# ApricityXX/PaddlePaddle

Hardware: AMD Instinct MI355X
Metric: tokens/sec GPT-3-13B sharding-3 + ResNet50 img/s, at 1/2/4/8 MI355X (higher is better)
Workload: dtype bf16; 1 GPU; model=GPT-3 13B (h5120 L40 a40 ffn20480 V50304), global_batch=16, seq_len=2048, micro_batch=4, accum_steps=4, parallelism=sharding_stage3_degree1, recompute=False, fused_head_ce=False, paired_wgrad=False, optimizer=AdamW fp32-master fused HIP, amp=O2 bf16, allocator=native auto-growth best-fit

## Files before the change

### csrc/dispatch/dispatch_gen.inc

```

extern "C" int pa_rms_norm_fwd(void*, void*, void*, void*, int64_t, int64_t, float, int, void*);
static PyObject* w_pa_rms_norm_fwd(PyObject*, PyObject* const* a, Py_ssize_t n) {
  if (n != 9) return bad_nargs("pa_rms_norm_fwd", 9, n);
  void* a0;
  if (!arg_ptr(a[0], &a0)) return nullptr;
  void* a1;
  if (!arg_ptr(a[1], &a1)) return nullptr;
  void* a2;
  if (!arg_ptr(a[2], &a2)) return nullptr;
  void* a3;
  if (!arg_ptr(a[3], &a3)) return nullptr;
  int64_t a4;
  if (!arg_i64(a[4], &a4)) return nullptr;
  int64_t a5;
  if (!arg_i64(a[5], &a5)) return nullptr;
  float a6;
  if (!arg_f32(a[6], &a6)) return nullptr;
  int a7;
  if (!arg_i32(a[7], &a7)) return nullptr;
  void* a8;
  if (!arg_ptr(a[8], &a8)) return nullptr;
  return PyLong_FromLongLong(static_cast<long long>(pa_rms_norm_fwd(a0, a1, a2, a3, a4, a5, a6, a7, a8)));
}
extern "C" int pa_rms_norm_bwd(void*, void*, void*, void*, void*, void*, int64_t, int64_t, int, void*);
// ... 116 lines not shown
  void* a2;
  if (!arg_ptr(a[2], &a2)) return nullptr;
  void* a3;
  if (!arg_ptr(a[3], &a3)) return nullptr;
  int a4;
  if (!arg_i32(a[4], &a4)) return nullptr;
  int64_t a5;
  if (!arg_i64(a[5], &a5)) return nullptr;
  int a6;
  if (!arg_i32(a[6], &a6)) return nullptr;
  int a7;
  if (!arg_i32(a[7], &a7)) return nullptr;
  void* a8;
  if (!arg_ptr(a[8], &a8)) return nullptr;
  return PyLong_FromLongLong(static_cast<long long>(pa_reduce_parts(a0, a1, a2, a3, a4, a5, a6, a7, a8)));
}
extern "C" int pa_softmax_fwd(void*, void*, int64_t, int64_t, int, void*);
static PyObject* w_pa_softmax_fwd(PyObject*, PyObject* const* a, Py_ssize_t n) {
  if (n != 6) return bad_nargs("pa_softmax_fwd", 6, n);
  void* a0;
  if (!arg_ptr(a[0], &a0)) return nullptr;
  void* a1;
  if (!arg_ptr(a[1], &a1)) return nullptr;
  int64_t a2;
  if (!arg_i64(a[2], &a2)) return nullptr;
  int64_t a3;
  if (!arg_i64(a[3], &a3)) return nullptr;
  int a4;
  if (!arg_i32(a[4], &a4)) return nullptr;
  void* a5;
// ... 2460 lines not shown
  if (!arg_ptr(a[6], &a6)) return nullptr;
  return PyLong_FromLongLong(static_cast<long long>(pa_moe_route(a0, a1, a2, a3, a4, a5, a6)));
}
extern "C" int pa_version();
static PyObject* w_pa_version(PyObject*, PyObject* const* a, Py_ssize_t n) {
  if (n != 0) return bad_nargs("pa_version", 0, n);
  return PyLong_FromLongLong(static_cast<long long>(pa_version()));
}
static PyMethodDef kGenMethods[] = {
    {"pa_rms_norm_fwd", reinterpret_cast<PyCFunction>(reinterpret_cast<void (*)(void)>(w_pa_rms_norm_fwd)), METH_FASTCALL, nullptr},
    {"pa_rms_norm_bwd", reinterpret_cast<PyCFunction>(reinterpret_cast<void (*)(void)>(w_pa_rms_norm_bwd)), METH_FASTCALL, nullptr},
    {"pa_rms_norm_bwd_res", reinterpret_cast<PyCFunction>(reinterpret_cast<void (*)(void)>(w_pa_rms_norm_bwd_res)), METH_FASTCALL, nullptr},
    {"pa_layer_norm_fwd", reinterpret_cast<PyCFunction>(reinterpret_cast<void (*)(void)>(w_pa_layer_norm_fwd)), METH_FASTCALL, nullptr},
    {"pa_layer_norm_bwd", reinterpret_cast<PyCFunction>(reinterpret_cast<void (*)(void)>(w_pa_layer_norm_bwd)), METH_FASTCALL, nullptr},
    {"pa_reduce_parts", reinterpret_cast<PyCFunction>(reinterpret_cast<void (*)(void)>(w_pa_reduce_parts)), METH_FASTCALL, nullptr},
    {"pa_softmax_fwd", reinterpret_cast<PyCFunction>(reinterpret_cast<void (*)(void)>(w_pa_softmax_fwd)), METH_FASTCALL, nullptr},
    {"pa_softmax_bwd", reinterpret_cast<PyCFunction>(reinterpret_cast<void (*)(void)>(w_pa_softmax_bwd)), METH_FASTCALL, nullptr},
    {"pa_softmax_ce_fwd", reinterpret_cast<PyCFunction>(reinterpret_cast<void (*)(void)>(w_pa_softmax_ce_fwd)), METH_FASTCALL, nullptr},
    {"pa_softmax_ce_bwd", reinterpret_cast<PyCFunction>(reinterpret_cast<void (*)(void)>(w_pa_softmax_ce_bwd)), METH_FASTCALL, nullptr},
    {"pa_ce_slice_fwd", reinterpret_cast<PyCFunction>(reinterpret_cast<void (*)(void)>(w_pa_ce_slice_fwd)), METH_FASTCALL, nullptr},
    {"pa_ce_slice_bwd", reinterpret_cast<PyCFunction>(reinterpret_cast<void (*)(void)>(w_pa_ce_slice_bwd)), METH_FASTCALL, nullptr},
    {"pa_gelu_fwd", reinterpret_cast<PyCFunction>(reinterpret_cast<void (*)(void)>(w_pa_gelu_fwd)), METH_FASTCALL, nullptr},
    {"pa_gelu_bwd", reinterpret_cast<PyCFunction>(reinterpret_cast<void (*)(void)>(w_pa_gelu_bwd)), METH_FASTCALL, nullptr},
    {"pa_swiglu_fwd", reinterpret_cast<PyCFunction>(reinterpret_cast<void (*)(void)>(w_pa_swiglu_fwd)), METH_FASTCALL, nullptr},
    {"pa_swiglu_bwd", reinterpret_cast<PyCFunction>(reinterpret_cast<void (*)(void)>(w_pa_swiglu_bwd)), METH_FASTCALL, nullptr},
    {"pa_bias_gelu_fwd", reinterpret_cast<PyCFunction>(reinterpret_cast<void (*)(void)>(w_pa_bias_gelu_fwd)), METH_FASTCALL, nullptr},
    {"pa_rope_fwd", reinterpret_cast<PyCFunction>(reinterpret_cast<void (*)(void)>(w_pa_rope_fwd)), METH_FASTCALL, nullptr},
    {"pa_rope_rows", reinterpret_cast<PyCFunction>(reinterpret_cast<void (*)(void)>(w_pa_rope_rows)), METH_FASTCALL, nullptr},
    {"pa_adamw_multi", reinterpret_cast<PyCFunction>(reinterpret_cast<void (*)(void)>(w_pa_adamw_multi)), METH_FASTCALL, nullptr},
    {"pa_adam_hyper_step", reinterpret_cast<PyCFunction>(reinterpret_cast<void (*)(void)>(w_pa_adam_hyper_step)), METH_FASTCALL, nullptr},
// ... 81 lines not shown
```

### csrc/kernels/common.h

```cpp
#pragma once
#include <hip/hip_runtime.h>
#include <hip/hip_bf16.h>
#include <hip/hip_fp16.h>
#include <stdint.h>

#define PA_EXPORT extern "C" __attribute__((visibility("default")))

namespace pa {

constexpr int kWave = 64;

enum DType : int { kF32 = 0, kF16 = 1, kBF16 = 2 };

using bf16 = __hip_bfloat16;
using f16 = __half;

template <typename T> struct Vec8;
template <> struct Vec8<bf16> { using type = uint4; };
template <> struct Vec8<f16> { using type = uint4; };

__device__ __forceinline__ float to_f(float x) { return x; }
__device__ __forceinline__ float to_f(bf16 x) { return __bfloat162float(x); }
__device__ __forceinline__ float to_f(f16 x) { return __half2float(x); }

// ... 100 lines not shown
template <int NT>
__device__ __forceinline__ float block_max(float v, float* smem) {
  v = wave_max(v);
  const int w = threadIdx.x >> 6, l = threadIdx.x & 63;
  __syncthreads();
  if (l == 0) smem[w] = v;
  __syncthreads();
  float r = -INFINITY;
#pragma unroll
  for (int i = 0; i < NT / 64; ++i) r = fmaxf(r, smem[i]);
  return r;
}

__host__ __device__ inline int64_t cdiv(int64_t a, int64_t b) { return (a + b - 1) / b; }

}

#define PA_DISPATCH_DTYPE(code, T, ...)                   \
  switch (code) {                                         \
    case pa::kF32: { using T = float; __VA_ARGS__; break; } \
    case pa::kF16: { using T = pa::f16; __VA_ARGS__; break; } \
    case pa::kBF16: { using T = pa::bf16; __VA_ARGS__; break; } \
    default: return 2;                                    \
  }

#define PA_CHECK_LAUNCH() do { hipError_t e_ = hipGetLastError(); if (e_ != hipSuccess) return 1; } while (0)
```

### csrc/kernels/linear_epi.hip

```cpp
#include "common.h"

using namespace pa;

namespace {

constexpr float kSqrt2OverPi = 0.7978845608028654f;
constexpr float kCoeff = 0.044715f;

__device__ __forceinline__ float gelu_tanh_grad(float x) { return gelu_tanh_grad_fast(x); }

__device__ __forceinline__ uint32_t hash32(uint64_t seed, uint64_t i) {
  uint64_t z = seed + (i + 1) * 0x9E3779B97F4A7C15ull;
  z = (z ^ (z >> 30)) * 0xBF58476D1CE4E5B9ull;
  z = (z ^ (z >> 27)) * 0x94D049BB133111EBull;
  z ^= z >> 31;
  return (uint32_t)(z >> 32);
}
__device__ __forceinline__ bool keep(uint64_t seed, uint64_t i, uint32_t thresh) { return hash32(seed, i) >= thresh; }

template <typename T>
__global__ __launch_bounds__(256) void colsum_partial_k(const T* __restrict__ x, float* __restrict__ part, int64_t rows,
                                                        int64_t cols, int nparts) {
  const int64_t c = ((int64_t)blockIdx.x * 256 + threadIdx.x) * 8;
  if (c >= cols) return;
  float acc[8] = {0, 0, 0, 0, 0, 0, 0, 0};
  for (int64_t r = blockIdx.y; r < rows; r += nparts) {
    float v[8];
    load8<T>(x + r * cols + c, v);
#pragma unroll
    for (int j = 0; j < 8; ++j) acc[j] += v[j];
  }
  store8<float>(part + (int64_t)blockIdx.y * cols + c, acc);
}
// ... 143 lines not shown
  const int dtype = dtype_acc & 0xff, acc = (dtype_acc >> 8) & 1;
  const int np = nparts_for(rows);
  dim3 g1((unsigned)cdiv(cols, 2048), (unsigned)np), g2((unsigned)cdiv(cols, 64));
  PA_DISPATCH_DTYPE(dtype, T, {
    hipLaunchKernelGGL((bias_gelu_bwd_k<T>), g1, dim3(256), 0, st, (const T*)h, (const T*)b, (const T*)dy, (T*)dh,
                       ws, rows, cols, np);
    hipLaunchKernelGGL((fold_partials_k<T>), g2, dim3(256), 0, st, ws, (T*)db, cols, np, acc);
  });
  PA_CHECK_LAUNCH();
  return 0;
}

PA_EXPORT int pa_dropout_add_fwd(const void* x, const void* res, void* out, int64_t n, float p, uint64_t seed,
                                 int dtype, hipStream_t st) {
  const int64_t nvec = n / 8;
  const uint32_t thresh = (uint32_t)fminf(p * 4294967296.0f, 4294967295.0f);
  const float scale = p < 1.f ? 1.f / (1.f - p) : 0.f;
  PA_DISPATCH_DTYPE(dtype, T, hipLaunchKernelGGL((dropout_add_k<T>), dim3(grid_ew(nvec)), dim3(256), 0, st,
                                                 (const T*)x, (const T*)res, (T*)out, nvec, seed, thresh, scale));
  PA_CHECK_LAUNCH();
  return 0;
}

PA_EXPORT int pa_dropout_bwd(const void* dy, void* dx, int64_t n, float p, uint64_t seed, int dtype, hipStream_t st) {
  const int64_t nvec = n / 8;
  const uint32_t thresh = (uint32_t)fminf(p * 4294967296.0f, 4294967295.0f);
  const float scale = p < 1.f ? 1.f / (1.f - p) : 0.f;
  PA_DISPATCH_DTYPE(dtype, T, hipLaunchKernelGGL((dropout_bwd_k<T>), dim3(grid_ew(nvec)), dim3(256), 0, st,
                                                 (const T*)dy, (T*)dx, nvec, seed, thresh, scale));
  PA_CHECK_LAUNCH();
  return 0;
}

PA_EXPORT int pa_dropout_bwd_colsum(const void* dy, void* dx, float* ws, int64_t rows, int64_t cols, float p,
                                    uint64_t seed, int dtype, hipStream_t st) {
  if (cols % 8) return 1;
  const uint32_t thresh = (uint32_t)fminf(p * 4294967296.0f, 4294967295.0f);
  const float scale = p < 1.f ? 1.f / (1.f - p) : 0.f;
  const int np = nparts_for(rows);
  dim3 g1((unsigned)cdiv(cols, 2048), (unsigned)np);
  PA_DISPATCH_DTYPE(dtype, T, hipLaunchKernelGGL((dropout_bwd_colsum_k<T>), g1, dim3(256), 0, st, (const T*)dy, (T*)dx,
                                                 ws, rows, cols, np, seed, thresh, scale));
  PA_CHECK_LAUNCH();
  return 0;
}

PA_EXPORT int64_t pa_colsum_nparts(int64_t rows) { return nparts_for(rows); }

PA_EXPORT int pa_fold_partials(const float* ws, void* out, int64_t cols, int64_t nparts, int dtype_acc,
                               hipStream_t st) {
  const int dtype = dtype_acc & 0xff, acc = (dtype_acc >> 8) & 1;
  dim3 g2((unsigned)cdiv(cols, 64));
  PA_DISPATCH_DTYPE(dtype, T, hipLaunchKernelGGL((fold_partials_k<T>), g2, dim3(256), 0, st, ws, (T*)out, cols,
// ... 5 lines not shown
```

### csrc/kernels/norm.hip

```cpp
#include "common.h"

using namespace pa;

namespace {

template <typename T, int VPL, bool LN>
__global__ __launch_bounds__(256) void norm_fwd_rows(const T* __restrict__ x, const T* __restrict__ w,
                                                     const T* __restrict__ b, T* __restrict__ y,
                                                     float* __restrict__ mean_out, float* __restrict__ rstd_out,
                                                     int64_t rows, int64_t cols, float eps) {
  const int lane = threadIdx.x & 63;
  const int64_t row = (int64_t)blockIdx.x * 4 + (threadIdx.x >> 6);
  if (row >= rows) return;
  const T* xr = x + row * cols;
  const float sh = LN ? to_f(xr[0]) : 0.f;
  float v[VPL][8];
  float s = 0.f;
#pragma unroll
  for (int k = 0; k < VPL; ++k) {
    const int64_t e = ((int64_t)k * 64 + lane) * 8;
    if (e < cols) {
      load8<T>(xr + e, v[k]);
    } else {
#pragma unroll
// ... 234 lines not shown
  else if (vpl <= 3) PA_BWD(3);
  else if (vpl <= 4) PA_BWD(4);
  else if (vpl <= 6) PA_BWD(6);
  else hipLaunchKernelGGL((norm_bwd_dx_wide<T, LN>), dim3((unsigned)rows), block, 0, st, DY, X, W, mean, rstd, DX, rows, cols,
                          RES);
#undef PA_BWD
  PA_CHECK_LAUNCH();
  if (dw_part) {
    dim3 g2((unsigned)cdiv(cols, 2048), (unsigned)nparts);
    hipLaunchKernelGGL((norm_bwd_wb<T, LN>), g2, block, 0, st, DY, X, mean, rstd, dw_part, db_part, rows, cols, nparts);
    PA_CHECK_LAUNCH();
  }
  return 0;
}

}

PA_EXPORT int pa_rms_norm_fwd(const void* x, const void* w, void* y, float* rstd, int64_t rows, int64_t cols,
                              float eps, int dtype, hipStream_t st) {
  PA_DISPATCH_DTYPE(dtype, T, return (launch_fwd<T, false>(x, w, nullptr, y, nullptr, rstd, rows, cols, eps, st)));
  return 0;
}

PA_EXPORT int pa_rms_norm_bwd(const void* dy, const void* x, const void* w, const float* rstd, void* dx,
                              float* dw_part, int64_t rows, int64_t cols, int dtype_np, hipStream_t st) {
  const int dtype = dtype_np & 0xff, nparts = dtype_np >> 8;
  PA_DISPATCH_DTYPE(dtype, T,
                    return (launch_bwd<T, false>(dy, x, w, nullptr, rstd, dx, w ? dw_part : nullptr, nullptr, rows,
                                                 cols, nparts > 0 ? nparts : 1, st)));
  return 0;
// ... 71 lines not shown
```

### paddlepaddle_amd/framework/flags.py

```python
from __future__ import annotations

import os

_FLAGS = {
    "FLAGS_check_nan_inf": False,
    "FLAGS_check_nan_inf_level": 0,
    "FLAGS_use_hip_kernels": True,
    "FLAGS_cudnn_deterministic": False,
    "FLAGS_embedding_deterministic": 0,
    "FLAGS_fraction_of_gpu_memory_to_use": 0.92,
    "FLAGS_allocator_strategy": "auto_growth",
    "FLAGS_eager_delete_tensor_gb": 0.0,
    "FLAGS_use_cuda_graph": False,
    "FLAGS_enable_pir_api": False,
    "FLAGS_print_ir": False,
    "FLAGS_call_stack_level": 1,
    "FLAGS_dp_bucket_mb": 128,
    "FLAGS_sharding_bucket_mb": 256,
    "FLAGS_pir_native_interpreter": True,
    "FLAGS_eager_backward_engine": "native",
    "FLAGS_weight_only_dequant_cache_mb": 4096,
    "FLAGS_fused_grad_accumulation": True,
    "FLAGS_static_native_executor": "auto",
    "FLAGS_gemm_backend": "auto",
    "FLAGS_sharding_stage3_keep_params": "auto",
    "FLAGS_conv_per_direction": True,
    "FLAGS_conv_bn_fusion": True,
    "FLAGS_use_autotune": True,
    "FLAGS_autotune_range_begin": 0,
    "FLAGS_autotune_range_end": 1 << 30,
    "FLAGS_layout_autotune": False,
    "FLAGS_dataloader_autotune": False,
    "FLAGS_dataloader_tuning_steps": 8,
    "FLAGS_static_engine_native": "auto",
    "FLAGS_linear_wt_cache_mb": 0,
}

for _k in list(_FLAGS):
    if _k in os.environ:
        _v = os.environ[_k]
        _d = _FLAGS[_k]
        if isinstance(_d, bool):
            _FLAGS[_k] = _v.lower() in ("1", "true", "yes")
        elif isinstance(_d, int):
            _FLAGS[_k] = int(_v)
        elif isinstance(_d, float):
            _FLAGS[_k] = float(_v)
        else:
            _FLAGS[_k] = _v

# ... 25 lines not shown
```

### paddlepaddle_amd/models/gpt.py

```python
from __future__ import annotations

import dataclasses
import math

import torch

from .. import nn
from ..framework.tensor import Tensor, _wrap
from ..nn import functional as F
from ..nn import initializer as I
from .. import ops as _ops


@dataclasses.dataclass
class GPTConfig:
    vocab_size: int = 50304
    hidden_size: int = 5120
    num_hidden_layers: int = 40
    num_attention_heads: int = 40
    intermediate_size: int = 20480
    max_position_embeddings: int = 2048
    hidden_dropout_prob: float = 0.1
    attention_probs_dropout_prob: float = 0.0
    initializer_range: float = 0.02
# ... 71 lines not shown
        init = I.Normal(0.0, cfg.initializer_range)
        if cfg.tensor_parallel_degree > 1:
            self.word_embeddings = _tp().VocabParallelEmbedding(cfg.vocab_size, cfg.hidden_size,
                                                                weight_attr=nn.ParamAttr(initializer=init))
        else:
            self.word_embeddings = nn.Embedding(cfg.vocab_size, cfg.hidden_size,
                                                weight_attr=nn.ParamAttr(initializer=init))
        self.position_embeddings = nn.Embedding(cfg.max_position_embeddings, cfg.hidden_size,
                                                weight_attr=nn.ParamAttr(initializer=init))
        self.dropout = nn.Dropout(cfg.hidden_dropout_prob)

        self.sp = _use_sp(cfg)
        if self.sp:
            _sp().mark_sequence_parallel(self.position_embeddings.weight)

    def forward(self, input_ids, position_ids=None):
        if self.sp:
            return self._forward_sp(input_ids, position_ids)
        if position_ids is None:
            S = input_ids.shape[-1]
            position_ids = _wrap(torch.arange(S, device=input_ids._t.device).unsqueeze(0))
        x = self.word_embeddings(input_ids)._t
        pe = self.position_embeddings(position_ids)._t
        p = self.dropout.p if self.training else 0.0
        return _wrap(_ops.dropout_add(x + pe, None, p, self.training))

    def _forward_sp(self, input_ids, position_ids):
        sp = _sp()
        ids = input_ids._t
        B, S = ids.shape[0], ids.shape[-1]
        emb = self.word_embeddings.local_lookup(ids).reshape(B * S, -1)
        x = sp.reduce_scatter_tokens(emb)
        r0, r1 = sp.token_block_range(B * S)
        if position_ids is None:
            pos = torch.arange(r0, r1, device=ids.device) % S
        else:
            pos = position_ids._t.expand(B, S).reshape(-1)[r0:r1]
        pe = torch.nn.functional.embedding(pos, self.position_embeddings.weight._t)
        p = self.dropout.p if self.training else 0.0
# ... 45 lines not shown
        return fn(qkv)

    def _forward_sp(self, x):
        sp = _sp()
        B, S = self.bs
        w, b = self.qkv_proj.weight._t, self.qkv_proj.bias._t
        t = x._t if x._t.dtype == w.dtype else x._t.to(w.dtype)
        qkv = sp.column_sp_linear(t, w, b)
        qkv = qkv.view(B, S, self.local_heads, 3, self.head_dim)
        o = _ops.flash_attention_qkvpacked(qkv, causal=True, dropout=self.attn_dropout, training=self.training)
        o = o.reshape(B * S, self.local_heads * self.head_dim)
        y = sp.row_sp_linear(o, self.out_proj.weight._t)
        return _wrap(y + self.out_proj.bias._t)


def _tracing():
    from ..framework.trace_hook import _active_program
    return _active_program() is not None


class GPTMLP(nn.Layer):
    def __init__(self, cfg: GPTConfig):
        super().__init__()
        h, f = cfg.hidden_size, cfg.intermediate_size
        init = I.Normal(0.0, cfg.initializer_range)
        out_init = I.Normal(0.0, cfg.initializer_range / math.sqrt(2.0 * cfg.num_hidden_layers))
        self.tp = cfg.tensor_parallel_degree
        if self.tp > 1:
            tp = _tp()
            self.linear1 = tp.ColumnParallelLinear(h, f, weight_attr=nn.ParamAttr(initializer=init), has_bias=True,
# ... 32 lines not shown


class GPTDecoderLayer(nn.Layer):
    def __init__(self, cfg: GPTConfig):
        super().__init__()
        self.norm1 = nn.LayerNorm(cfg.hidden_size, epsilon=cfg.layer_norm_eps)
        self.self_attn = GPTAttention(cfg)
        self.norm2 = nn.LayerNorm(cfg.hidden_size, epsilon=cfg.layer_norm_eps)
        self.mlp = GPTMLP(cfg)
        self.dropout1 = nn.Dropout(cfg.hidden_dropout_prob)
        self.dropout2 = nn.Dropout(cfg.hidden_dropout_prob)
        if _use_sp(cfg):
            _sp().mark_sequence_parallel(self.norm1.weight, self.norm1.bias, self.norm2.weight, self.norm2.bias)

    def _ln(self, norm, x):
        r, h = _ops.layer_norm_residual(x._t, norm.weight._t, norm.bias._t, norm._epsilon)
        return r, _wrap(h)

    def _attn(self, h):
        return _gpt_attn(self, h)

    def forward(self, x):
        p = self.dropout1.p if self.training else 0.0
        r, h = self._ln(self.norm1, x)
        x = _wrap(_ops.dropout_add(self._attn(h)._t, r, p, self.training))
        r, h = self._ln(self.norm2, x)
        x = _wrap(_ops.dropout_add(self.mlp(h)._t, r, p, self.training))
        return x


def _gpt_attn(layer, h):
    g = getattr(layer, "_rc", None)
    if g == "full_attn":
        from ..distributed.fleet.recompute import recompute
        return recompute(layer.self_attn, h)
    layer.self_attn._rc_core = g == "core_attn"
    return layer.self_attn(h)


class GPTModel(nn.Layer):
    def __init__(self, cfg: GPTConfig):
        super().__init__()
        self.config = cfg
        self.embeddings = GPTEmbeddings(cfg)
        self.layers = nn.LayerList([GPTDecoderLayer(cfg) for _ in range(cfg.num_hidden_layers)])
        self.norm = nn.LayerNorm(cfg.hidden_size, epsilon=cfg.layer_norm_eps)
        if _use_sp(cfg):
            _sp().mark_sequence_parallel(self.norm.weight, self.norm.bias)

    def forward(self, input_ids, position_ids=None):
        if _use_sp(self.config):
            bs = (input_ids.shape[0], input_ids.shape[-1])
            for layer in self.layers:
                layer.self_attn.bs = bs
        x = self.embeddings(input_ids, position_ids)
        rc = self.config.use_recompute and self.training
        gran = self.config.recompute_granularity
        skip = set(self.config.no_recompute_layers or ())
        if rc:
            from ..distributed.fleet.recompute import recompute
        for i, layer in enumerate(self.layers):
            on = rc and i not in skip
            if on and gran == "full":
                x = recompute(layer, x)
            else:
                layer._rc = gran if on else None
                x = layer(x)
        return self.norm(x)


class GPTForPretraining(nn.Layer):
    def __init__(self, cfg: GPTConfig):
        super().__init__()
        self.config = cfg
        self.gpt = GPTModel(cfg)
        if not cfg.tie_word_embeddings:
            self.lm_head_weight = self.create_parameter([cfg.vocab_size // max(cfg.tensor_parallel_degree, 1),
                                                         cfg.hidden_size],
                                                        default_initializer=I.Normal(0.0, cfg.initializer_range))

    def forward(self, input_ids, position_ids=None, labels=None, loss_mask=None, ignore_index=-100):
        h = self.gpt(input_ids, position_ids)
# ... 42 lines not shown
```

### paddlepaddle_amd/ops/__init__.py

```python
from __future__ import annotations

from .activation import gelu, silu, swiglu, softmax, bias_gelu
from .norm import rms_norm, rms_norm_residual, layer_norm, layer_norm_residual, add_rms_norm
from .loss import softmax_cross_entropy
from .attention import flash_attention, attention_bhsd, flash_attention_qkvpacked, qkv_rope_attention, attention_reference, paged_decode_attention, dense_decode_attention
from .rope import apply_rotary, decode_rope_cache
from .linear import fused_linear, colsum, linear_nt, ffn_gelu
from .lm_head import lm_head_cross_entropy
from .dropout import dropout_add
from . import optim
from ._loader import has as has_kernel, hip_enabled_for, LIB_PATH
from .bn import batch_norm_act_nhwc
from . import conv, gemm, dwconv, quant
```

### paddlepaddle_amd/ops/_sigs.py

```python
import ctypes

_vp = ctypes.c_void_p
_i64 = ctypes.c_int64
_i32 = ctypes.c_int
_f32 = ctypes.c_float
_u64 = ctypes.c_uint64

SIGS = {
    "pa_rms_norm_fwd": [_vp, _vp, _vp, _vp, _i64, _i64, _f32, _i32, _vp],
    "pa_rms_norm_bwd": [_vp, _vp, _vp, _vp, _vp, _vp, _i64, _i64, _i32, _vp],
    "pa_rms_norm_bwd_res": [_vp, _vp, _vp, _vp, _vp, _vp, _vp, _i64, _i64, _i32, _vp],
    "pa_layer_norm_fwd": [_vp, _vp, _vp, _vp, _vp, _vp, _i64, _i64, _f32, _i32, _vp],
    "pa_layer_norm_bwd": [_vp, _vp, _vp, _vp, _vp, _vp, _vp, _vp, _vp, _i64, _i64, _i32, _vp],
    "pa_reduce_parts": [_vp, _vp, _vp, _vp, _i32, _i64, _i32, _i32, _vp],
    "pa_softmax_fwd": [_vp, _vp, _i64, _i64, _i32, _vp],
    "pa_softmax_bwd": [_vp, _vp, _vp, _i64, _i64, _i32, _vp],
    "pa_softmax_ce_fwd": [_vp, _vp, _vp, _vp, _i64, _i64, _i64, _i32, _vp],
    "pa_softmax_ce_bwd": [_vp, _vp, _vp, _vp, _vp, _i64, _i64, _i64, _i32, _vp],
    "pa_ce_slice_fwd": [_vp, _vp, _vp, _vp, _i64, _i64, _i64, _i32, _vp],
    "pa_ce_slice_bwd": [_vp, _vp, _vp, _vp, _vp, _i64, _i64, _i64, _i64, _i32, _vp],
    "pa_gelu_fwd": [_vp, _vp, _i64, _i32, _i32, _vp],
    "pa_gelu_bwd": [_vp, _vp, _vp, _i64, _i32, _i32, _vp],
    "pa_swiglu_fwd": [_vp, _vp, _vp, _i64, _i64, _i64, _i32, _vp],
    "pa_swiglu_bwd": [_vp, _vp, _vp, _vp, _vp, _i64, _i64, _i64, _i32, _vp],
    "pa_bias_gelu_fwd": [_vp, _vp, _vp, _i64, _i64, _i32, _vp],
    "pa_rope_fwd": [_vp, _vp, _vp, _vp, _i64, _i64, _i64, _i64, _i32, _i32, _vp],
    "pa_rope_rows": [_vp, _i64, _vp, _vp, _vp, _i64, _i64, _i64, _i64, _i64, _i32, _i32, _vp],
    "pa_adamw_multi": [_vp, _vp, _i64, _vp, _f32, _f32, _f32, _f32, _f32, _f32, _f32, _vp, _vp],
    "pa_adam_hyper_step": [_vp, _f32, _f32, _vp],
# ... 81 lines not shown
    "pa_bn_bwd_apply_nhwc": [_vp] * 6 + [_i64, _i32, _i32, _vp, _vp],
    "pa_bn_pre_ws": [_i32, _i32],
    "pa_bn_bwd_nhwc_pre": [_vp] * 9 + [_i32, _vp, _vp, _i64, _i32, _i32, _vp, _vp],
    "pa_bn_fwd_nhwc_pre": [_vp] * 10 + [_i32, _vp, _vp, _vp, _i64, _i32, _f32, _f32, _i32, _vp],
    "pa_add_rms_norm_fwd": [_vp, _vp, _vp, _vp, _vp, _i64, _i64, _f32, _i32, _vp],
    "pa_decode_rope_cache": [_vp, _i64, _vp, _vp, _vp, _vp, _vp, _vp, _i32, _i32, _i32, _i32, _i64, _i32, _vp],
    "pa_maxpool_nhwc_fwd": [_vp, _vp, _vp] + [_i32] * 10 + [_vp],
    "pa_maxpool_nhwc_bwd": [_vp, _vp, _vp] + [_i32] * 10 + [_vp],
    "pa_grouped_gemm": [_i32, _vp, _vp, _vp, _vp, _vp, _vp, _i32, _i64, _i32, _i32, _i32, _i64, _i64, _i64, _i32,
                        _vp],
    "pa_moe_route": [_vp, _i32, _i32, _vp, _vp, _vp, _vp],
    "pa_version": [],
}

RET_I64 = {"pa_flash_attn_bwd_ds_bytes", "pa_gemm_pp_ws_bytes", "pa_gemm_fp8_ws_bytes", "pa_gemm_pp_splitk_ws_bytes", "pa_bn_pre_ws", "pa_gemm_skinny_stats_chunks", "pa_conv_skinny_stats_chunks",
           "pa_colsum_nparts", "pa_multi_tensor_chunk"}
```

Baseline: 13950 tokens/s.

## Fuse dropout-add with the following LayerNorm in GPT forward and backward

Adds HIP kernels that fuse the residual dropout-add with the next LayerNorm. The forward kernel writes both the residual sum and the normalized output. The backward kernel computes the LayerNorm gradient, applies the dropout mask, and optionally accumulates column partials. GPT layers now defer dropout_add as a pending tensor that the next norm consumes, which removes separate elementwise passes over the hidden activations. It is enabled by default when sequence parallelism, recompute and tracing are off. The cost is extra model-level plumbing and a different backward partial-reduction path.

```diff
diff --git a/csrc/dispatch/dispatch_gen.inc b/csrc/dispatch/dispatch_gen.inc
--- a/csrc/dispatch/dispatch_gen.inc
+++ b/csrc/dispatch/dispatch_gen.inc
@@ -154,6 +154,87 @@
   void* a8;
   if (!arg_ptr(a[8], &a8)) return nullptr;
   return PyLong_FromLongLong(static_cast<long long>(pa_reduce_parts(a0, a1, a2, a3, a4, a5, a6, a7, a8)));
+}
+extern "C" int pa_dropout_add_layer_norm_fwd(void*, void*, void*, void*, void*, void*, void*, void*, int64_t, int64_t, float, float, uint64_t, int, void*);
+static PyObject* w_pa_dropout_add_layer_norm_fwd(PyObject*, PyObject* const* a, Py_ssize_t n) {
+  if (n != 15) return bad_nargs("pa_dropout_add_layer_norm_fwd", 15, n);
+  void* a0;
+  if (!arg_ptr(a[0], &a0)) return nullptr;
+  void* a1;
+  if (!arg_ptr(a[1], &a1)) return nullptr;
+  void* a2;
+  if (!arg_ptr(a[2], &a2)) return nullptr;
+  void* a3;
+  if (!arg_ptr(a[3], &a3)) return nullptr;
+  void* a4;
+  if (!arg_ptr(a[4], &a4)) return nullptr;
+  void* a5;
+  if (!arg_ptr(a[5], &a5)) return nullptr;
+  void* a6;
+  if (!arg_ptr(a[6], &a6)) return nullptr;
+  void* a7;
+  if (!arg_ptr(a[7], &a7)) return nullptr;
+  int64_t a8;
+  if (!arg_i64(a[8], &a8)) return nullptr;
+  int64_t a9;
+  if (!arg_i64(a[9], &a9)) return nullptr;
+  float a10;
+  if (!arg_f32(a[10], &a10)) return nullptr;
+  float a11;
+  if (!arg_f32(a[11], &a11)) return nullptr;
+  uint64_t a12;
+  if (!arg_u64(a[12], &a12)) return nullptr;
+  int a13;
+  if (!arg_i32(a[13], &a13)) return nullptr;
+  void* a14;
+  if (!arg_ptr(a[14], &a14)) return nullptr;
+  return PyLong_FromLongLong(static_cast<long long>(pa_dropout_add_layer_norm_fwd(a0, a1, a2, a3, a4, a5, a6, a7, a8, a9, a10, a11, a12, a13, a14)));
+}
+extern "C" int pa_layer_norm_bwd_dropout(void*, void*, void*, void*, void*, void*, void*, void*, void*, void*, void*, int64_t, int64_t, float, uint64_t, int, void*);
+static PyObject* w_pa_layer_norm_bwd_dropout(PyObject*, PyObject* const* a, Py_ssize_t n) {
+  if (n != 17) return bad_nargs("pa_layer_norm_bwd_dropout", 17, n);
+  void* a0;
+  if (!arg_ptr(a[0], &a0)) return nullptr;
+  void* a1;
+  if (!arg_ptr(a[1], &a1)) return nullptr;
+  void* a2;
+  if (!arg_ptr(a[2], &a2)) return nullptr;
+  void* a3;
+  if (!arg_ptr(a[3], &a3)) return nullptr;
+  void* a4;
+  if (!arg_ptr(a[4], &a4)) return nullptr;
+  void* a5;
+  if (!arg_ptr(a[5], &a5)) return nullptr;
+  void* a6;
+  if (!arg_ptr(a[6], &a6)) return nullptr;
+  void* a7;
+  if (!arg_ptr(a[7], &a7)) return nullptr;
+  void* a8;
+  if (!arg_ptr(a[8], &a8)) return nullptr;
+  void* a9;
+  if (!arg_ptr(a[9], &a9)) return nullptr;
+  void* a10;
+  if (!arg_ptr(a[10], &a10)) return nullptr;
+  int64_t a11;
+  if (!arg_i64(a[11], &a11)) return nullptr;
+  int64_t a12;
+  if (!arg_i64(a[12], &a12)) return nullptr;
+  float a13;
+  if (!arg_f32(a[13], &a13)) return nullptr;
+  uint64_t a14;
+  if (!arg_u64(a[14], &a14)) return nullptr;
+  int a15;
+  if (!arg_i32(a[15], &a15)) return nullptr;
+  void* a16;
+  if (!arg_ptr(a[16], &a16)) return nullptr;
+  return PyLong_FromLongLong(static_cast<long long>(pa_layer_norm_bwd_dropout(a0, a1, a2, a3, a4, a5, a6, a7, a8, a9, a10, a11, a12, a13, a14, a15, a16)));
+}
+extern "C" int64_t pa_layer_norm_bwd_dropout_grid(int64_t);
+static PyObject* w_pa_layer_norm_bwd_dropout_grid(PyObject*, PyObject* const* a, Py_ssize_t n) {
+  if (n != 1) return bad_nargs("pa_layer_norm_bwd_dropout_grid", 1, n);
+  int64_t a0;
+  if (!arg_i64(a[0], &a0)) return nullptr;
+  return PyLong_FromLongLong(static_cast<long long>(pa_layer_norm_bwd_dropout_grid(a0)));
 }
 extern "C" int pa_softmax_fwd(void*, void*, int64_t, int64_t, int, void*);
 static PyObject* w_pa_softmax_fwd(PyObject*, PyObject* const* a, Py_ssize_t n) {
@@ -2644,6 +2725,9 @@
     {"pa_layer_norm_fwd", reinterpret_cast<PyCFunction>(reinterpret_cast<void (*)(void)>(w_pa_layer_norm_fwd)), METH_FASTCALL, nullptr},
     {"pa_layer_norm_bwd", reinterpret_cast<PyCFunction>(reinterpret_cast<void (*)(void)>(w_pa_layer_norm_bwd)), METH_FASTCALL, nullptr},
     {"pa_reduce_parts", reinterpret_cast<PyCFunction>(reinterpret_cast<void (*)(void)>(w_pa_reduce_parts)), METH_FASTCALL, nullptr},
+    {"pa_dropout_add_layer_norm_fwd", reinterpret_cast<PyCFunction>(reinterpret_cast<void (*)(void)>(w_pa_dropout_add_layer_norm_fwd)), METH_FASTCALL, nullptr},
+    {"pa_layer_norm_bwd_dropout", reinterpret_cast<PyCFunction>(reinterpret_cast<void (*)(void)>(w_pa_layer_norm_bwd_dropout)), METH_FASTCALL, nullptr},
+    {"pa_layer_norm_bwd_dropout_grid", reinterpret_cast<PyCFunction>(reinterpret_cast<void (*)(void)>(w_pa_layer_norm_bwd_dropout_grid)), METH_FASTCALL, nullptr},
     {"pa_softmax_fwd", reinterpret_cast<PyCFunction>(reinterpret_cast<void (*)(void)>(w_pa_softmax_fwd)), METH_FASTCALL, nullptr},
     {"pa_softmax_bwd", reinterpret_cast<PyCFunction>(reinterpret_cast<void (*)(void)>(w_pa_softmax_bwd)), METH_FASTCALL, nullptr},
     {"pa_softmax_ce_fwd", reinterpret_cast<PyCFunction>(reinterpret_cast<void (*)(void)>(w_pa_softmax_ce_fwd)), METH_FASTCALL, nullptr},
diff --git a/csrc/kernels/common.h b/csrc/kernels/common.h
--- a/csrc/kernels/common.h
+++ b/csrc/kernels/common.h
@@ -138,6 +138,17 @@
 
 __host__ __device__ inline int64_t cdiv(int64_t a, int64_t b) { return (a + b - 1) / b; }
 
+__device__ __forceinline__ uint32_t hash32(uint64_t seed, uint64_t i) {
+  uint64_t z = seed + (i + 1) * 0x9E3779B97F4A7C15ull;
+  z = (z ^ (z >> 30)) * 0xBF58476D1CE4E5B9ull;
+  z = (z ^ (z >> 27)) * 0x94D049BB133111EBull;
+  z ^= z >> 31;
+  return (uint32_t)(z >> 32);
+}
+__device__ __forceinline__ bool keep(uint64_t seed, uint64_t i, uint32_t thresh) { return hash32(seed, i) >= thresh; }
+inline uint32_t dropout_thresh(float p) { return (uint32_t)fminf(p * 4294967296.0f, 4294967295.0f); }
+inline float dropout_scale(float p) { return p < 1.f ? 1.f / (1.f - p) : 0.f; }
+
 }
 
 #define PA_DISPATCH_DTYPE(code, T, ...)                   \
diff --git a/csrc/kernels/linear_epi.hip b/csrc/kernels/linear_epi.hip
--- a/csrc/kernels/linear_epi.hip
+++ b/csrc/kernels/linear_epi.hip
@@ -9,14 +9,6 @@
 
 __device__ __forceinline__ float gelu_tanh_grad(float x) { return gelu_tanh_grad_fast(x); }
 
-__device__ __forceinline__ uint32_t hash32(uint64_t seed, uint64_t i) {
-  uint64_t z = seed + (i + 1) * 0x9E3779B97F4A7C15ull;
-  z = (z ^ (z >> 30)) * 0xBF58476D1CE4E5B9ull;
-  z = (z ^ (z >> 27)) * 0x94D049BB133111EBull;
-  z ^= z >> 31;
-  return (uint32_t)(z >> 32);
-}
-__device__ __forceinline__ bool keep(uint64_t seed, uint64_t i, uint32_t thresh) { return hash32(seed, i) >= thresh; }
 
 template <typename T>
 __global__ __launch_bounds__(256) void colsum_partial_k(const T* __restrict__ x, float* __restrict__ part, int64_t rows,
@@ -190,8 +182,8 @@
 PA_EXPORT int pa_dropout_add_fwd(const void* x, const void* res, void* out, int64_t n, float p, uint64_t seed,
                                  int dtype, hipStream_t st) {
   const int64_t nvec = n / 8;
-  const uint32_t thresh = (uint32_t)fminf(p * 4294967296.0f, 4294967295.0f);
-  const float scale = p < 1.f ? 1.f / (1.f - p) : 0.f;
+  const uint32_t thresh = dropout_thresh(p);
+  const float scale = dropout_scale(p);
   PA_DISPATCH_DTYPE(dtype, T, hipLaunchKernelGGL((dropout_add_k<T>), dim3(grid_ew(nvec)), dim3(256), 0, st,
                                                  (const T*)x, (const T*)res, (T*)out, nvec, seed, thresh, scale));
   PA_CHECK_LAUNCH();
@@ -200,8 +192,8 @@
 
 PA_EXPORT int pa_dropout_bwd(const void* dy, void* dx, int64_t n, float p, uint64_t seed, int dtype, hipStream_t st) {
   const int64_t nvec = n / 8;
-  const uint32_t thresh = (uint32_t)fminf(p * 4294967296.0f, 4294967295.0f);
-  const float scale = p < 1.f ? 1.f / (1.f - p) : 0.f;
+  const uint32_t thresh = dropout_thresh(p);
+  const float scale = dropout_scale(p);
   PA_DISPATCH_DTYPE(dtype, T, hipLaunchKernelGGL((dropout_bwd_k<T>), dim3(grid_ew(nvec)), dim3(256), 0, st,
                                                  (const T*)dy, (T*)dx, nvec, seed, thresh, scale));
   PA_CHECK_LAUNCH();
@@ -211,8 +203,8 @@
 PA_EXPORT int pa_dropout_bwd_colsum(const void* dy, void* dx, float* ws, int64_t rows, int64_t cols, float p,
                                     uint64_t seed, int dtype, hipStream_t st) {
   if (cols % 8) return 1;
-  const uint32_t thresh = (uint32_t)fminf(p * 4294967296.0f, 4294967295.0f);
-  const float scale = p < 1.f ? 1.f / (1.f - p) : 0.f;
+  const uint32_t thresh = dropout_thresh(p);
+  const float scale = dropout_scale(p);
   const int np = nparts_for(rows);
   dim3 g1((unsigned)cdiv(cols, 2048), (unsigned)np);
   PA_DISPATCH_DTYPE(dtype, T, hipLaunchKernelGGL((dropout_bwd_colsum_k<T>), g1, dim3(256), 0, st, (const T*)dy, (T*)dx,
diff --git a/csrc/kernels/norm.hip b/csrc/kernels/norm.hip
--- a/csrc/kernels/norm.hip
+++ b/csrc/kernels/norm.hip
@@ -272,6 +272,332 @@
   return 0;
 }
 
+template <typename T> __device__ __forceinline__ uint4 pack8(const float* f);
+template <> __device__ __forceinline__ uint4 pack8<bf16>(const float* f) {
+  return make_uint4(pack_bf16(f[0], f[1]), pack_bf16(f[2], f[3]), pack_bf16(f[4], f[5]), pack_bf16(f[6], f[7]));
+}
+template <> __device__ __forceinline__ uint4 pack8<f16>(const float* f) {
+  return make_uint4(pack_f16(f[0], f[1]), pack_f16(f[2], f[3]), pack_f16(f[4], f[5]), pack_f16(f[6], f[7]));
+}
+template <typename T> __device__ __forceinline__ void unpack8(uint4 v, float* f);
+template <> __device__ __forceinline__ void unpack8<bf16>(uint4 v, float* f) {
+  f[0] = lo_bf16(v.x); f[1] = hi_bf16(v.x); f[2] = lo_bf16(v.y); f[3] = hi_bf16(v.y);
+  f[4] = lo_bf16(v.z); f[5] = hi_bf16(v.z); f[6] = lo_bf16(v.w); f[7] = hi_bf16(v.w);
+}
+template <> __device__ __forceinline__ void unpack8<f16>(uint4 v, float* f) {
+  f[0] = lo_f16(v.x); f[1] = hi_f16(v.x); f[2] = lo_f16(v.y); f[3] = hi_f16(v.y);
+  f[4] = lo_f16(v.z); f[5] = hi_f16(v.z); f[6] = lo_f16(v.w); f[7] = hi_f16(v.w);
+}
+template <typename T> __device__ __forceinline__ uint32_t pack2(float a, float b);
+template <> __device__ __forceinline__ uint32_t pack2<bf16>(float a, float b) { return pack_bf16(a, b); }
+template <> __device__ __forceinline__ uint32_t pack2<f16>(float a, float b) { return pack_f16(a, b); }
+template <typename T> __device__ __forceinline__ void unpack2(uint32_t v, float* f);
+template <> __device__ __forceinline__ void unpack2<bf16>(uint32_t v, float* f) { f[0] = lo_bf16(v); f[1] = hi_bf16(v); }
+template <> __device__ __forceinline__ void unpack2<f16>(uint32_t v, float* f) { f[0] = lo_f16(v); f[1] = hi_f16(v); }
+__device__ __forceinline__ uint4 ld16(const void* p) { return *reinterpret_cast<const uint4*>(p); }
+__device__ __forceinline__ void st16(void* p, uint4 v) { *reinterpret_cast<uint4*>(p) = v; }
+
+template <typename T, bool DROP>
+__device__ __forceinline__ void drop_add8(const T* __restrict__ z, const T* __restrict__ r, T* __restrict__ x,
+                                          int64_t e, uint64_t seed, uint32_t thresh, float scale, float* v) {
+  float a[8];
+  load8<T>(z + e, a);
+  if (r) load8<T>(r + e, v); else {
+#pragma unroll
+    for (int j = 0; j < 8; ++j) v[j] = 0.f;
+  }
+#pragma unroll
+  for (int j = 0; j < 8; ++j) {
+    if (DROP) v[j] += keep(seed, e + j, thresh) ? a[j] * scale : 0.f;
+    else v[j] += a[j];
+  }
+  const uint4 q = pack8<T>(v);
+  st16(x + e, q);
+  unpack8<T>(q, v);
+}
+
+template <typename T, int VPL, bool DROP>
+__global__ __launch_bounds__(256) void dropout_add_ln_fwd_rows(const T* __restrict__ z, const T* __restrict__ r,
+                                                               const T* __restrict__ w, const T* __restrict__ b,
+                                                               T* __restrict__ x, T* __restrict__ y,
+                                                               float* __restrict__ mean_out, float* __restrict__ rstd_out,
+                                                               int64_t rows, int64_t cols, float eps, uint64_t seed,
+                                                               uint32_t thresh, float scale) {
+  const int lane = threadIdx.x & 63;
+  const int64_t row = (int64_t)blockIdx.x * 4 + (threadIdx.x >> 6);
+  if (row >= rows) return;
+  float v[VPL][8];
+#pragma unroll
+  for (int k = 0; k < VPL; ++k) {
+    const int64_t e = ((int64_t)k * 64 + lane) * 8;
+    if (e < cols) drop_add8<T, DROP>(z, r, x, row * cols + e, seed, thresh, scale, v[k]);
+  }
+  const float sh = __shfl(v[0][0], 0, 64);
+  float s = 0.f;
+#pragma unroll
+  for (int k = 0; k < VPL; ++k) {
+    const int64_t e = ((int64_t)k * 64 + lane) * 8;
+    if (e >= cols) {
+#pragma unroll
+      for (int j = 0; j < 8; ++j) v[k][j] = sh;
+    }
+#pragma unroll
+    for (int j = 0; j < 8; ++j) s += v[k][j] - sh;
+  }
+  s = wave_sum(s);
+  const float inv_n = 1.0f / (float)cols;
+  const float mu = sh + s * inv_n;
+  float s2 = 0.f;
+#pragma unroll
+  for (int k = 0; k < VPL; ++k) {
+    const int64_t e = ((int64_t)k * 64 + lane) * 8;
+    if (e < cols) {
+#pragma unroll
+      for (int j = 0; j < 8; ++j) { float d = v[k][j] - mu; s2 += d * d; }
+    }
+  }
+  s2 = wave_sum(s2);
+  const float rstd = rsqrtf(s2 * inv_n + eps);
+  if (lane == 0) {
+    mean_out[row] = mu;
+    rstd_out[row] = rstd;
+  }
+  T* yr = y + row * cols;
+#pragma unroll
+  for (int k = 0; k < VPL; ++k) {
+    const int64_t e = ((int64_t)k * 64 + lane) * 8;
+    if (e < cols) {
+      float o[8], wv[8], bv[8];
+      load8<T>(w + e, wv);
+      load8<T>(b + e, bv);
+#pragma unroll
+      for (int j = 0; j < 8; ++j) o[j] = (v[k][j] - mu) * rstd * wv[j] + bv[j];
+      store8<T>(yr + e, o);
+    }
+  }
+}
+
+template <typename T, int NV, bool DROP>
+__global__ __launch_bounds__(256) void dropout_add_ln_fwd_wide(const T* __restrict__ z, const T* __restrict__ r,
+                                                               const T* __restrict__ w, const T* __restrict__ b,
+                                                               T* __restrict__ x, T* __restrict__ y,
+                                                               float* __restrict__ mean_out, float* __restrict__ rstd_out,
+                                                               int64_t rows, int64_t cols, float eps, uint64_t seed,
+                                                               uint32_t thresh, float scale) {
+  __shared__ float red[4];
+  __shared__ float first;
+  const int64_t row = blockIdx.x;
+  float v[NV][8];
+#pragma unroll
+  for (int k = 0; k < NV; ++k) {
+    const int64_t e = (int64_t)threadIdx.x * 8 + k * 2048;
+    if (e < cols) drop_add8<T, DROP>(z, r, x, row * cols + e, seed, thresh, scale, v[k]);
+  }
+  if (threadIdx.x == 0) first = v[0][0];
+  __syncthreads();
+  const float sh = first;
+  float s = 0.f, s2 = 0.f;
+#pragma unroll
+  for (int k = 0; k < NV; ++k) {
+    const int64_t e = (int64_t)threadIdx.x * 8 + k * 2048;
+    if (e < cols) {
+#pragma unroll
+      for (int j = 0; j < 8; ++j) { const float d = v[k][j] - sh; s += d; s2 += d * d; }
+    }
+  }
+  const float inv_n = 1.0f / (float)cols;
+  s = block_sum<256>(s, red);
+  s2 = block_sum<256>(s2, red);
+  const float md = s * inv_n;
+  const float mu = sh + md;
+  const float rstd = rsqrtf(fmaxf(s2 * inv_n - md * md, 0.f) + eps);
+  if (threadIdx.x == 0) {
+    mean_out[row] = mu;
+    rstd_out[row] = rstd;
+  }
+  T* yr = y + row * cols;
+#pragma unroll
+  for (int k = 0; k < NV; ++k) {
+    const int64_t e = (int64_t)threadIdx.x * 8 + k * 2048;
+    if (e < cols) {
+      float o[8], wv[8], bv[8];
+      load8<T>(w + e, wv);
+      load8<T>(b + e, bv);
+#pragma unroll
+      for (int j = 0; j < 8; ++j) o[j] = (v[k][j] - mu) * rstd * wv[j] + bv[j];
+      store8<T>(yr + e, o);
+    }
+  }
+}
+
+template <typename T, bool DROP>
+__global__ __launch_bounds__(1024) void ln_bwd_dropout_k(const T* __restrict__ dy, const T* __restrict__ x,
+                                                         const T* __restrict__ w, const float* __restrict__ mean,
+                                                         const float* __restrict__ rstd, const T* __restrict__ res,
+                                                         T* __restrict__ dx, T* __restrict__ dz, float* __restrict__ pw,
+                                                         float* __restrict__ pb, float* __restrict__ pz, int64_t rows,
+                                                         int64_t cols, uint64_t seed, uint32_t thresh, float scale) {
+  __shared__ float red[2][16];
+  const int wave = threadIdx.x >> 6, lane = threadIdx.x & 63, nwave = blockDim.x >> 6;
+  const int64_t e = (int64_t)threadIdx.x * 8;
+  const bool on = e < cols;
+  float aw[8], ab[8], az[8];
+#pragma unroll
+  for (int j = 0; j < 8; ++j) aw[j] = ab[j] = az[j] = 0.f;
+  uint4 xq = make_uint4(0, 0, 0, 0), dq = xq, wq = xq;
+  if (on && (int64_t)blockIdx.x < rows) {
+    wq = ld16(w + e);
+    xq = ld16(x + (int64_t)blockIdx.x * cols + e);
+    dq = ld16(dy + (int64_t)blockIdx.x * cols + e);
+  }
+  const float inv_n = 1.0f / (float)cols;
+  for (int64_t row = blockIdx.x; row < rows; row += gridDim.x) {
+    const int64_t next = row + gridDim.x, f = row * cols + e;
+    uint4 xn = xq, dn = dq, rq = xq;
+    if (on) {
+      if (res) rq = ld16(res + f);
+      if (next < rows) {
+        xn = ld16(x + next * cols + e);
+        dn = ld16(dy + next * cols + e);
+      }
+    }
+    const float mu = mean[row], rs = rstd[row];
+    float sg = 0.f, sgx = 0.f;
+    if (on) {
+      float xv[8], dv[8], wv[8];
+      unpack8<T>(xq, xv);
+      unpack8<T>(dq, dv);
+      unpack8<T>(wq, wv);
+#pragma unroll
+      for (int j = 0; j < 8; ++j) { float gg = dv[j] * wv[j]; sg += gg; sgx += gg * (xv[j] - mu) * rs; }
+    }
+    asm volatile("" : "+v"(xq.x), "+v"(xq.y), "+v"(xq.z), "+v"(xq.w), "+v"(dq.x), "+v"(dq.y), "+v"(dq.z), "+v"(dq.w));
+    sgx = wave_sum(sgx);
+    sg = wave_sum(sg);
+    __syncthreads();
+    if (lane == 0) { red[0][wave] = sgx; red[1][wave] = sg; }
+    __syncthreads();
+    sgx = 0.f, sg = 0.f;
+    for (int i = 0; i < nwave; ++i) { sgx += red[0][i]; sg += red[1][i]; }
+    sgx *= inv_n;
+    sg *= inv_n;
+    if (on) {
+      const uint32_t xw[4] = {xq.x, xq.y, xq.z, xq.w}, dw[4] = {dq.x, dq.y, dq.z, dq.w};
+      const uint32_t ww[4] = {wq.x, wq.y, wq.z, wq.w}, rw[4] = {rq.x, rq.y, rq.z, rq.w};
+      uint32_t ow[4], zw[4];
+#pragma unroll
+      for (int i = 0; i < 4; ++i) {
+        float xv[2], dv[2], wv[2], rv[2], o[2];
+        unpack2<T>(xw[i], xv);
+        unpack2<T>(dw[i], dv);
+        unpack2<T>(ww[i], wv);
+        unpack2<T>(rw[i], rv);
+#pragma unroll
+        for (int j = 0; j < 2; ++j) {
+          const float xh = (xv[j] - mu) * rs;
+          o[j] = rs * (dv[j] * wv[j] - sg - xh * sgx);
+          if (res) o[j] += rv[j];
+          aw[2 * i + j] += dv[j] * (xv[j] - mu) * rs;
+          ab[2 * i + j] += dv[j];
+        }
+        ow[i] = pack2<T>(o[0], o[1]);
+        unpack2<T>(ow[i], o);
+#pragma unroll
+        for (int j = 0; j < 2; ++j) {
+          if (DROP) o[j] = keep(seed, f + 2 * i + j, thresh) ? o[j] * scale : 0.f;
+          az[2 * i + j] += o[j];
+        }
+        if (DROP) zw[i] = pack2<T>(o[0], o[1]);
+      }
+      st16(dx + f, make_uint4(ow[0], ow[1], ow[2], ow[3]));
+      if (DROP) st16(dz + f, make_uint4(zw[0], zw[1], zw[2], zw[3]));
+    }
+    xq = xn;
+    dq = dn;
+  }
+  if (on && (int64_t)blockIdx.x < rows) {
+    store8<float>(pw + (int64_t)blockIdx.x * cols + e, aw);
+    store8<float>(pb + (int64_t)blockIdx.x * cols + e, ab);
+    if (pz) store8<float>(pz + (int64_t)blockIdx.x * cols + e, az);
+  }
+}
+
+inline int64_t bwd_dropout_grid(int64_t rows) { return rows < 512 ? (rows < 1 ? 1 : rows) : 512; }
+
+constexpr int64_t kFusedMaxCols = 8192;
+
+template <typename T, bool DROP>
+int launch_dropout_add_ln_fwd(const void* z, const void* r, const void* w, const void* b, void* x, void* y, float* mean,
+                              float* rstd, int64_t rows, int64_t cols, float eps, uint64_t seed, uint32_t thresh,
+                              float scale, hipStream_t st) {
+  const int64_t vpl = cdiv(cols, 512), nv = cdiv(cols, 2048);
+  dim3 grid((unsigned)cdiv(rows, 4)), block(256);
+#define PA_ARGS (const T*)z, (const T*)r, (const T*)w, (const T*)b, (T*)x, (T*)y, mean, rstd, rows, cols, eps, seed, thresh, scale
+#define PA_ROWS(V) hipLaunchKernelGGL((dropout_add_ln_fwd_rows<T, V, DROP>), grid, block, 0, st, PA_ARGS)
+#define PA_WIDE(V) hipLaunchKernelGGL((dropout_add_ln_fwd_wide<T, V, DROP>), dim3((unsigned)rows), block, 0, st, PA_ARGS)
+  if (vpl <= 1) PA_ROWS(1);
+  else if (vpl <= 2) PA_ROWS(2);
+  else if (vpl <= 3) PA_ROWS(3);
+  else if (vpl <= 4) PA_ROWS(4);
+  else if (vpl <= 6) PA_ROWS(6);
+  else if (nv <= 2) PA_WIDE(2);
+  else if (nv <= 3) PA_WIDE(3);
+  else PA_WIDE(4);
+#undef PA_WIDE
+#undef PA_ROWS
+#undef PA_ARGS
+  PA_CHECK_LAUNCH();
+  return 0;
+}
+
+template <typename T, bool DROP>
+int launch_ln_bwd_dropout(const void* dy, const void* x, const void* w, const float* mean, const float* rstd,
+                          const void* res, void* dx, void* dz, float* pw, float* pb, float* pz, int64_t rows,
+                          int64_t cols, uint64_t seed, uint32_t thresh, float scale, hipStream_t st) {
+  dim3 grid((unsigned)bwd_dropout_grid(rows)), block((unsigned)(cdiv(cols, 512) * 64));
+  hipLaunchKernelGGL((ln_bwd_dropout_k<T, DROP>), grid, block, 0, st, (const T*)dy, (const T*)x, (const T*)w, mean, rstd,
+                     (const T*)res, (T*)dx, (T*)dz, pw, pb, pz, rows, cols, seed, thresh, scale);
+  PA_CHECK_LAUNCH();
+  return 0;
+}
+
+}
+
+PA_EXPORT int pa_dropout_add_layer_norm_fwd(const void* z, const void* r, const void* w, const void* b, void* x,
+                                            void* h, float* mean, float* rstd, int64_t rows, int64_t cols, float eps,
+                                            float p, uint64_t seed, int dtype, hipStream_t st) {
+  if (cols % 8 || cols > kFusedMaxCols || cols < 8 || rows < 1 || !w || !b) return 3;
+  const uint32_t thresh = dropout_thresh(p);
+  const float scale = dropout_scale(p);
+#define PA_GO(T)                                                                                                    \
+  return p > 0.f ? launch_dropout_add_ln_fwd<T, true>(z, r, w, b, x, h, mean, rstd, rows, cols, eps, seed, thresh,  \
+                                                      scale, st)                                                    \
+                 : launch_dropout_add_ln_fwd<T, false>(z, r, w, b, x, h, mean, rstd, rows, cols, eps, seed, thresh, \
+                                                       scale, st)
+  if (dtype == kBF16) PA_GO(bf16);
+  if (dtype == kF16) PA_GO(f16);
+#undef PA_GO
+  return 2;
+}
+
+PA_EXPORT int64_t pa_layer_norm_bwd_dropout_grid(int64_t rows) { return bwd_dropout_grid(rows); }
+
+PA_EXPORT int pa_layer_norm_bwd_dropout(const void* dh, const void* x, const void* w, const float* mean,
+                                        const float* rstd, const void* g_res, void* dx, void* dz, float* pw, float* pb,
+                                        float* pz, int64_t rows, int64_t cols, float p, uint64_t seed, int dtype,
+                                        hipStream_t st) {
+  if (cols % 8 || cols > kFusedMaxCols || cols < 8 || rows < 1 || !w) return 3;
+  const uint32_t thresh = dropout_thresh(p);
+  const float scale = dropout_scale(p);
+#define PA_GO(T)                                                                                                     \
+  return p > 0.f ? launch_ln_bwd_dropout<T, true>(dh, x, w, mean, rstd, g_res, dx, dz, pw, pb, pz, rows, cols, seed, \
+                                                  thresh, scale, st)                                                 \
+                 : launch_ln_bwd_dropout<T, false>(dh, x, w, mean, rstd, g_res, dx, dz, pw, pb, pz, rows, cols,      \
+                                                   seed, thresh, scale, st)
+  if (dtype == kBF16) PA_GO(bf16);
+  if (dtype == kF16) PA_GO(f16);
+#undef PA_GO
+  return 2;
 }
 
 PA_EXPORT int pa_rms_norm_fwd(const void* x, const void* w, void* y, float* rstd, int64_t rows, int64_t cols,
diff --git a/paddlepaddle_amd/framework/flags.py b/paddlepaddle_amd/framework/flags.py
--- a/paddlepaddle_amd/framework/flags.py
+++ b/paddlepaddle_amd/framework/flags.py
@@ -34,6 +34,7 @@
     "FLAGS_dataloader_tuning_steps": 8,
     "FLAGS_static_engine_native": "auto",
     "FLAGS_linear_wt_cache_mb": 0,
+    "FLAGS_fused_dropout_add_ln": True,
 }
 
 for _k in list(_FLAGS):
diff --git a/paddlepaddle_amd/models/gpt.py b/paddlepaddle_amd/models/gpt.py
--- a/paddlepaddle_amd/models/gpt.py
+++ b/paddlepaddle_amd/models/gpt.py
@@ -109,7 +109,7 @@
         if self.sp:
             _sp().mark_sequence_parallel(self.position_embeddings.weight)
 
-    def forward(self, input_ids, position_ids=None):
+    def forward(self, input_ids, position_ids=None, defer_dropout=False):
         if self.sp:
             return self._forward_sp(input_ids, position_ids)
         if position_ids is None:
@@ -118,6 +118,8 @@
         x = self.word_embeddings(input_ids)._t
         pe = self.position_embeddings(position_ids)._t
         p = self.dropout.p if self.training else 0.0
+        if defer_dropout:
+            return _pending(x + pe, None, p)
         return _wrap(_ops.dropout_add(x + pe, None, p, self.training))
 
     def _forward_sp(self, input_ids, position_ids):
@@ -193,6 +195,21 @@
         return _wrap(y + self.out_proj.bias._t)
 
 
+def _pending(z, r, p):
+    t = _wrap(z)
+    t._pa_pending = (r, p)
+    return t
+
+
+def _is_pending(x):
+    return getattr(x, "_pa_pending", None) is not None
+
+
+def _fuse_dropout_add_ln(cfg):
+    from ..framework.flags import flag
+    return bool(flag("FLAGS_fused_dropout_add_ln", True)) and not _use_sp(cfg) and not _tracing()
+
+
 def _tracing():
     from ..framework.trace_hook import _active_program
     return _active_program() is not None
@@ -255,7 +272,12 @@
             _sp().mark_sequence_parallel(self.norm1.weight, self.norm1.bias, self.norm2.weight, self.norm2.bias)
 
     def _ln(self, norm, x):
-        r, h = _ops.layer_norm_residual(x._t, norm.weight._t, norm.bias._t, norm._epsilon)
+        if _is_pending(x):
+            res, p = x._pa_pending
+            r, h = _ops.dropout_add_layer_norm(x._t, res, norm.weight._t, norm.bias._t, p, self.training,
+                                               norm._epsilon)
+        else:
+            r, h = _ops.layer_norm_residual(x._t, norm.weight._t, norm.bias._t, norm._epsilon)
         return r, _wrap(h)
 
     def _attn(self, h):
@@ -263,11 +285,13 @@
 
     def forward(self, x):
         p = self.dropout1.p if self.training else 0.0
+        fused = _is_pending(x)
         r, h = self._ln(self.norm1, x)
-        x = _wrap(_ops.dropout_add(self._attn(h)._t, r, p, self.training))
+        z = self._attn(h)._t
+        x = _pending(z, r, p) if fused else _wrap(_ops.dropout_add(z, r, p, self.training))
         r, h = self._ln(self.norm2, x)
-        x = _wrap(_ops.dropout_add(self.mlp(h)._t, r, p, self.training))
-        return x
+        z = self.mlp(h)._t
+        return _pending(z, r, p) if fused else _wrap(_ops.dropout_add(z, r, p, self.training))
 
 
 def _gpt_attn(layer, h):
@@ -294,8 +318,10 @@
             bs = (input_ids.shape[0], input_ids.shape[-1])
             for layer in self.layers:
                 layer.self_attn.bs = bs
-        x = self.embeddings(input_ids, position_ids)
         rc = self.config.use_recompute and self.training
+        fused = not rc and _fuse_dropout_add_ln(self.config)
+        x = self.embeddings(input_ids, position_ids, defer_dropout=True) if fused else \
+            self.embeddings(input_ids, position_ids)
         gran = self.config.recompute_granularity
         skip = set(self.config.no_recompute_layers or ())
         if rc:
@@ -307,6 +333,11 @@
             else:
                 layer._rc = gran if on else None
                 x = layer(x)
+        if _is_pending(x):
+            res, p = x._pa_pending
+            _, h = _ops.dropout_add_layer_norm(x._t, res, self.norm.weight._t, self.norm.bias._t, p, self.training,
+                                               self.norm._epsilon)
+            return _wrap(h)
         return self.norm(x)
 
 
diff --git a/paddlepaddle_amd/ops/__init__.py b/paddlepaddle_amd/ops/__init__.py
--- a/paddlepaddle_amd/ops/__init__.py
+++ b/paddlepaddle_amd/ops/__init__.py
@@ -2,6 +2,7 @@
 
 from .activation import gelu, silu, swiglu, softmax, bias_gelu
 from .norm import rms_norm, rms_norm_residual, layer_norm, layer_norm_residual, add_rms_norm
+from .dropout_add_norm import dropout_add_layer_norm
 from .loss import softmax_cross_entropy
 from .attention import flash_attention, attention_bhsd, flash_attention_qkvpacked, qkv_rope_attention, attention_reference, paged_decode_attention, dense_decode_attention
 from .rope import apply_rotary, decode_rope_cache
diff --git a/paddlepaddle_amd/ops/_sigs.py b/paddlepaddle_amd/ops/_sigs.py
--- a/paddlepaddle_amd/ops/_sigs.py
+++ b/paddlepaddle_amd/ops/_sigs.py
@@ -13,6 +13,10 @@
     "pa_layer_norm_fwd": [_vp, _vp, _vp, _vp, _vp, _vp, _i64, _i64, _f32, _i32, _vp],
     "pa_layer_norm_bwd": [_vp, _vp, _vp, _vp, _vp, _vp, _vp, _vp, _vp, _i64, _i64, _i32, _vp],
     "pa_reduce_parts": [_vp, _vp, _vp, _vp, _i32, _i64, _i32, _i32, _vp],
+    "pa_dropout_add_layer_norm_fwd": [_vp, _vp, _vp, _vp, _vp, _vp, _vp, _vp, _i64, _i64, _f32, _f32, _u64, _i32, _vp],
+    "pa_layer_norm_bwd_dropout": [_vp, _vp, _vp, _vp, _vp, _vp, _vp, _vp, _vp, _vp, _vp, _i64, _i64, _f32, _u64, _i32,
+                                  _vp],
+    "pa_layer_norm_bwd_dropout_grid": [_i64],
     "pa_softmax_fwd": [_vp, _vp, _i64, _i64, _i32, _vp],
     "pa_softmax_bwd": [_vp, _vp, _vp, _i64, _i64, _i32, _vp],
     "pa_softmax_ce_fwd": [_vp, _vp, _vp, _vp, _i64, _i64, _i64, _i32, _vp],
@@ -124,4 +128,4 @@
 }
 
 RET_I64 = {"pa_flash_attn_bwd_ds_bytes", "pa_gemm_pp_ws_bytes", "pa_gemm_fp8_ws_bytes", "pa_gemm_pp_splitk_ws_bytes", "pa_bn_pre_ws", "pa_gemm_skinny_stats_chunks", "pa_conv_skinny_stats_chunks",
-           "pa_colsum_nparts", "pa_multi_tensor_chunk"}
+           "pa_colsum_nparts", "pa_multi_tensor_chunk", "pa_layer_norm_bwd_dropout_grid"}
diff --git a/paddlepaddle_amd/ops/dropout_add_norm.py b/paddlepaddle_amd/ops/dropout_add_norm.py
--- /dev/null
+++ b/paddlepaddle_amd/ops/dropout_add_norm.py
@@ -0,0 +1,63 @@
+from __future__ import annotations
+
+import torch
+
+from . import _loader as L
+from . import dropout as _dropout
+from .norm import _finalize_parts, layer_norm_residual
+
+MAX_COLS = 8192
+
+
+class _DropoutAddLayerNormFn(torch.autograd.Function):
+    @staticmethod
+    def forward(ctx, z, r, w, b, p, eps):
+        cols = z.shape[-1]
+        z2 = z.contiguous().view(-1, cols)
+        r2 = r.contiguous().to(z.dtype).view(-1, cols) if r is not None else None
+        rows = z2.shape[0]
+        x = torch.empty_like(z2)
+        h = torch.empty_like(z2)
+        mean = torch.empty(rows, dtype=torch.float32, device=z.device)
+        rstd = torch.empty(rows, dtype=torch.float32, device=z.device)
+        wc = w.contiguous().to(z.dtype)
+        bc = b.contiguous().to(z.dtype)
+        seed = _dropout._seed() if p > 0.0 else 0
+        L.call("pa_dropout_add_layer_norm_fwd", L.ptr(z2), L.ptr(r2), L.ptr(wc), L.ptr(bc), L.ptr(x), L.ptr(h),
+               L.ptr(mean), L.ptr(rstd), rows, cols, float(eps), float(p), seed, L.dcode(z2), L.stream_ptr())
+        ctx.save_for_backward(x, wc, mean, rstd)
+        ctx.seed, ctx.p, ctx.has_res = seed, p, r is not None
+        ctx.w_dtype, ctx.b_dtype, ctx.params, ctx.shape = w.dtype, b.dtype, (w, b), z.shape
+        return x.view(z.shape), h.view(z.shape)
+
+    @staticmethod
+    def backward(ctx, g_x, dh):
+        x2, wc, mean, rstd = ctx.saved_tensors
+        rows, cols = x2.shape
+        if g_x is None and dh is None:
+            return None, None, None, None, None, None
+        res = None if g_x is None else g_x.contiguous().view(rows, cols).to(x2.dtype)
+        dh2 = torch.zeros_like(x2) if dh is None else dh.contiguous().view(rows, cols).to(x2.dtype)
+        dx = torch.empty(ctx.shape, dtype=x2.dtype, device=x2.device)
+        dz = torch.empty_like(dx) if ctx.p > 0.0 else dx
+        grid = int(L.lib().pa_layer_norm_bwd_dropout_grid(rows))
+        parts = torch.empty(3, grid, cols, dtype=torch.float32, device=x2.device)
+        key = (rows, cols, x2.dtype)
+        want = key in _dropout._WANT_CS
+        L.call("pa_layer_norm_bwd_dropout", L.ptr(dh2), L.ptr(x2), L.ptr(wc), L.ptr(mean), L.ptr(rstd), L.ptr(res),
+               L.ptr(dx), L.ptr(dz), L.ptr(parts[0]), L.ptr(parts[1]), L.ptr(parts[2] if want else None), rows, cols,
+               float(ctx.p), ctx.seed, L.dcode(x2), L.stream_ptr())
+        dw, db = _finalize_parts(parts[0], parts[1], ctx.w_dtype, ctx.b_dtype, grid, cols, ctx.params)
+        dz._pa_cs_key, dz._pa_cs = key, ((parts[2], grid, dz._version) if want else None)
+        return dz, (dx if ctx.has_res else None), dw, db, None, None
+
+
+def dropout_add_layer_norm(z, r, gamma, beta, p, training=True, eps=1e-5):
+    p = float(p) if training else 0.0
+    cols = z.shape[-1]
+    if (L.hip_enabled_for(z) and z.dtype in (torch.bfloat16, torch.float16) and cols % 8 == 0 and cols <= MAX_COLS
+            and z.numel() > 0 and gamma is not None and beta is not None and (r is None or r.shape == z.shape)
+            and not (p == 0.0 and r is None)):
+        return _DropoutAddLayerNormFn.apply(z, r, gamma, beta, p, float(eps))
+    x = _dropout.dropout_add(z, r, p, training)
+    return layer_norm_residual(x, gamma, beta, eps)
```

Result: no change. 14010 tokens/s (median of 6 runs) (+0.4%).
